# Lalwaniamisha789/Implementation-of-Neural-LDPC-Decoders-with-Degree-Specific-Weight-Sharing-and-RCQ-Quantization

Measured on AMD Instinct MI355X. Metric: decoded codewords/sec at fixed iters; achieved HBM GB/s vs peak, higher is better.
Workload: dtype f32

## Files before the change

### implementation-of-neural-ldpc-decoders-with-degree-specific-weight-sharing-and-rcq-quantization_amd/csrc/ldpc_resident.hip

```cpp
#pragma once

#include "ldpc_kernels.hip"
#include "ldpc_resident_geom.h"

namespace ldpc {

struct ResidentPlan {
    int n, m, S, max_dc, max_dv;
    int mstride;
    const uint8_t *dc_s;
    const uint8_t *gsz;
    int any_split;
    int par_words;
    int par_shift;
    const uint16_t *cvar;
    const uint16_t *bslot;
    const uint16_t *bslot_c;
    const uint16_t *oaslot;
    const uint32_t *vmeta;
    const uint2 *vslot_lo;
    const uint2 *vslot_hi;
    int n_hi;
    const uint16_t *inv_perm_v;
    int n_pos;
// ... 722 lines not shown
        }
    }
}

__device__ __forceinline__ uint4 plan_unpack(const uint2 &p)
{
    return make_uint4(p.x & 0xffffu, p.x >> 16, p.y & 0xffffu, p.y >> 16);
}

template <int G, int MODE, typename T, int DMAX = 8>
__device__ __forceinline__ void res_var_dispatch(unsigned char *smem, T *__restrict__ llr_s,
                                                 uint8_t *__restrict__ bits_s, int q, int dv, const uint4 &slo,
                                                 const uint4 &shi, T a, unsigned emask, const ParScatter &ps,
                                                 Pack<T, G> *lreg = nullptr)
{
#define LDPC_RV(D) \
    case D: if constexpr (D <= DMAX) res_var_body<G, D, MODE, T>(smem, llr_s, bits_s, q, slo, shi, a, emask, ps, lreg); break;
    switch (dv) {
        LDPC_RV(0) LDPC_RV(1) LDPC_RV(2) LDPC_RV(3) LDPC_RV(4) LDPC_RV(5) LDPC_RV(6) LDPC_RV(7) LDPC_RV(8)
    default: break;
    }
#undef LDPC_RV
}

template <typename T, int G>
struct ResVarState {
    unsigned meta[kResRegVars];
    uint2 plo[kResRegVars];
    uint2 phi0;
    Pack<T, G> l[kResRegVars];
    unsigned cells;
};

template <int G, int MODE, typename T, int R>
__device__ __forceinline__ void res_var_round_cpt(const ResidentPlan &pl, unsigned char *smem, const T *__restrict__ alpha_glb,
                                                  unsigned emask, int tid, int nt, ResVarState<T, G> &st)
{
    constexpr int DMAX = R == 0 ? 8 : 4;
    const unsigned cd = (st.cells >> (8 * R)) & 0xffu;
    if (cd == kCellEmpty) return;
    const int q = tid + R * nt;
    const uint4 slo = plan_unpack(st.plo[R]), shi = R == 0 ? plan_unpack(st.phi0) : make_uint4(0, 0, 0, 0);
    T a = (T)0;
    if (MODE == 0) a = alpha_glb[pl.vmeta[q] >> 8];
    const ParScatter ps{};
    if (cd == kCellMixed) {
        res_var_dispatch<G, MODE, T, DMAX>(smem, nullptr, nullptr, q, (int)(pl.vmeta[q] & 0xffu), slo, shi, a, emask, ps,
                                           &st.l[R]);
        return;
    }
    if ((cd & kCellHoles) && st.plo[R].y == kResHole) return;
#define LDPC_RVU(D) \
    case D: if constexpr (D <= DMAX) res_var_body<G, D, MODE, T>(smem, nullptr, nullptr, q, slo, shi, a, emask, ps, &st.l[R]); break;
    switch (cd & 0xfu) {
        LDPC_RVU(1) LDPC_RVU(2) LDPC_RVU(3) LDPC_RVU(4) LDPC_RVU(5) LDPC_RVU(6) LDPC_RVU(7) LDPC_RVU(8)
    default: break;
    }
#undef LDPC_RVU
}

template <int G, int MODE, typename T>
__device__ __forceinline__ void res_var_phase_cpt(const ResidentPlan &pl, unsigned char *smem, const T *__restrict__ alpha_glb,
                                                  unsigned emask, int tid, int nt, ResVarState<T, G> &st)
{
#pragma unroll
    for (int r = 0; r < kResRegVars; ++r) asm volatile("" : "+v"(st.plo[r].x), "+v"(st.plo[r].y));
    asm volatile("" : "+v"(st.phi0.x), "+v"(st.phi0.y));
    static_assert(kResRegVars == 4, "four rounds");
    res_var_round_cpt<G, MODE, T, 0>(pl, smem, alpha_glb, emask, tid, nt, st);
    res_var_round_cpt<G, MODE, T, 1>(pl, smem, alpha_glb, emask, tid, nt, st);
    res_var_round_cpt<G, MODE, T, 2>(pl, smem, alpha_glb, emask, tid, nt, st);
    res_var_round_cpt<G, MODE, T, 3>(pl, smem, alpha_glb, emask, tid, nt, st);
}

template <int G, int MODE, typename T>
__device__ __forceinline__ void res_var_phase_reg(const ResidentPlan &pl, unsigned char *smem,
                                                  T *__restrict__ llr_s, uint8_t *__restrict__ bits_s,
                                                  const T *__restrict__ alpha_lds,
                                                  const T *__restrict__ alpha_glb, unsigned emask,
                                                  int tid, int nt, ResVarState<T, G> &st, const ParScatter &ps)
{
#pragma unroll
    for (int r = 0; r < kResRegVars; ++r) asm volatile("" : "+v"(st.meta[r]), "+v"(st.plo[r].x), "+v"(st.plo[r].y));
    asm volatile("" : "+v"(st.phi0.x), "+v"(st.phi0.y));
#pragma unroll
    for (int r = 0; r < kResRegVars; ++r) {
        const int q = tid + r * nt;
        if (__builtin_amdgcn_readfirstlane(q - (tid & 63)) >= pl.n) break;
        if (q < pl.n) {
            const unsigned meta = st.meta[r];
            const uint4 slo = plan_unpack(st.plo[r]), shi = r == 0 ? plan_unpack(st.phi0) : make_uint4(0, 0, 0, 0);
            T a = (T)0;
            if (MODE == 0 || MODE == 4) a = alpha_lds ? alpha_lds[meta >> 8] : alpha_glb[meta >> 8];
            res_var_dispatch<G, MODE, T>(smem, llr_s, bits_s, q, (int)(meta & 0xffu), slo, shi, a, emask, ps, &st.l[r]);
        }
    }
}

template <int G, int MODE, typename T, bool REG, bool CPT = false>
__device__ __forceinline__ void res_var_phase(const ResidentPlan &pl, unsigned char *smem,
                                              T *__restrict__ llr_s, uint8_t *__restrict__ bits_s,
                                              const T *__restrict__ alpha_lds,
                                              const T *__restrict__ alpha_glb, unsigned emask,
                                              int tid, int nt, ResVarState<T, G> &st,
                                              const ParScatter ps = ParScatter{})
{
    if constexpr (CPT) {
        static_assert(REG && (MODE == 0 || MODE == 2 || MODE == 9), "compact: fixed-T register-state modes");
        res_var_phase_cpt<G, MODE, T>(pl, smem, alpha_glb, emask, tid, nt, st);
        return;
    } else if constexpr (REG) {
        res_var_phase_reg<G, MODE, T>(pl, smem, llr_s, bits_s, alpha_lds, alpha_glb, emask, tid, nt, st, ps);
        return;
    }
    const int n = pl.n, n_hi = pl.n_hi;
    const int hi_last = (n_hi > 0 ? n_hi : 1) - 1;
    int q = tid;
    unsigned meta = 0;
    uint2 plo = make_uint2(0, 0), phi = make_uint2(0, 0);
    if (q < n) {
        meta = pl.vmeta[q];
        plo = pl.vslot_lo[q];
        phi = pl.vslot_hi[min(q, hi_last)];
    }
    while (q < n) {
        const int qn = q + nt;
        unsigned metan;
        uint2 plon, phin;
        {
            const unsigned qc = (unsigned)min(qn, n - 1), qh = min(qc, (unsigned)hi_last);
            metan = *reinterpret_cast<const uint32_t *>(reinterpret_cast<const char *>(pl.vmeta) + (size_t)(qc << 2));
            plon = *reinterpret_cast<const uint2 *>(reinterpret_cast<const char *>(pl.vslot_lo) + (size_t)(qc << 3));
            phin = *reinterpret_cast<const uint2 *>(reinterpret_cast<const char *>(pl.vslot_hi) + (size_t)(qh << 3));
        }
        const int dv = (int)(meta & 0xffu);
        const uint4 slo = plan_unpack(plo), shi = plan_unpack(phi);
        T a = (T)0;
        if (MODE == 0 || MODE == 4) a = alpha_lds ? alpha_lds[meta >> 8] : alpha_glb[meta >> 8];
        res_var_dispatch<G, MODE, T>(smem, llr_s, bits_s, q, dv, slo, shi, a, emask, ps);
        q = qn; meta = metan; plo = plon; phi = phin;
    }
}

template <int G, bool SPLIT>
__device__ __forceinline__ void res_syndrome_phase(const ResidentPlan &pl, const uint8_t *__restrict__ bits_s,
                                                   unsigned *sh_unsat, int tid, int nt)
{
    unsigned acc = 0;
    for (int p = tid; p < pl.m; p += nt) {
        const int dc = pl.dc_s[p];
        int dcw;
        unsigned x = 0;
        if (wave_uniform(dc, dcw)) {
#pragma unroll 8
            for (int t = 0; t < dcw; ++t) x ^= bits_s[pl.cvar[t * pl.mstride + p]];
        } else {
            for (int t = 0; t < dc; ++t) x ^= bits_s[pl.cvar[t * pl.mstride + p]];
        }
        if constexpr (SPLIT) x = group_xor(pl.gsz[p], x);
        acc |= x;
    }
    if (acc) atomicOr(sh_unsat, acc);
}

template <int G, bool SPLIT>
__device__ __forceinline__ void res_parity_reduce(const ResidentPlan &pl, unsigned par_off, unsigned *sh_unsat, int tid, int nt)
{
    unsigned acc = 0;
    for (int p = tid; p < pl.m; p += nt) {
        unsigned x = lds_load<unsigned>(par_off + 4u * (unsigned)p);
        lds_store<unsigned>(par_off + 4u * (unsigned)p, 0u);
        if constexpr (SPLIT) x = group_xor(pl.gsz[p], x);
        acc |= x;
    }
    if (acc) atomicOr(sh_unsat, acc);
}

template <int G, typename T, bool SPLIT>
__device__ __forceinline__ void res_syndrome_slots(const ResidentPlan &pl, unsigned *sh_unsat, int tid, int nt)
{
    constexpr unsigned kSlot = sizeof(Pack<T, G>);
    unsigned acc = 0;
    for (int p = tid; p < pl.m; p += nt) {
        const int dc = pl.dc_s[p];
        int dcw;
        unsigned x = 0;
        if (wave_uniform(dc, dcw)) {
            int t = 0;
#pragma unroll 4
            for (; t + 1 < dcw; t += 2)
                x = __builtin_amdgcn_bitop3_b32(x, lds_load<unsigned>((unsigned)(t * pl.mstride + p) * kSlot),
                                                lds_load<unsigned>((unsigned)((t + 1) * pl.mstride + p) * kSlot), 0x96);
            if (t < dcw) x ^= lds_load<unsigned>((unsigned)(t * pl.mstride + p) * kSlot);
        } else {
            for (int t = 0; t < dc; ++t) x ^= lds_load<unsigned>((unsigned)(t * pl.mstride + p) * kSlot);
        }
        if constexpr (SPLIT) x = group_xor(pl.gsz[p], x);
        acc |= x;
    }
    if (acc) atomicOr(sh_unsat, acc);
}

constexpr int kEmit = 4;

template <int G>
__device__ __forceinline__ void res_store_packed(const ResidentArgs &a, long long b, int j, int n, bool neg)
{
    const unsigned long long m = __ballot(neg);
    const int lane = threadIdx.x & 63;
    const int base = j - lane;
    if (lane < 8 && base + 8 * lane < n) a.packed[(size_t)b * ((n + 7) / 8) + (base >> 3) + lane] = (uint8_t)(m >> (8 * lane));
}

template <int G, typename T>
__device__ __forceinline__ void res_emit(const ResidentPlan &pl, const ResidentArgs &a, const T *__restrict__ llr_s,
                                         long long b0, unsigned mask, int iters, unsigned unsat, int tid, int nt)
{
    using P = Pack<T, G>;
    T *posterior = reinterpret_cast<T *>(a.posterior);
    const int n = pl.n;
    if (a.posterior || a.bits || a.packed) {
        for (int j0 = tid; j0 < n; j0 += kEmit * nt) {
            unsigned ip[kEmit];
#pragma unroll
            for (int k = 0; k < kEmit; ++k) ip[k] = (j0 + k * nt < n) ? pl.inv_perm_v[j0 + k * nt] : 0u;
#pragma unroll
            for (int k = 0; k < kEmit; ++k) {
                const int j = j0 + k * nt;
                if (j - (tid & 63) >= n) break;
                const bool in = j < n;
                const P p = reinterpret_cast<const P *>(llr_s)[ip[k]];
#pragma unroll
                for (int g = 0; g < G; ++g) {
                    if (!((mask >> g) & 1u)) continue;
                    if (in && a.posterior) res_stream_store(&posterior[(size_t)(b0 + g) * n + j], p.x[g]);
                    if (in && a.bits) res_stream_store(&a.bits[(size_t)(b0 + g) * n + j], p.x[g] < (T)0 ? 1 : 0);
                    if (a.packed) res_store_packed<G>(a, b0 + g, j, n, in && p.x[g] < (T)0);
                }
            }
        }
    }
    if (tid == 0) {
#pragma unroll
        for (int g = 0; g < G; ++g) {
            if (!((mask >> g) & 1u)) continue;
            if (a.iterations) a.iterations[b0 + g] = iters;
            if (a.success) a.success[b0 + g] = (uint8_t)(((unsat >> g) & 1u) ? 0 : 1);
        }
    }
}

template <int G>
__device__ __forceinline__ void res_emit_bits(const ResidentPlan &pl, const ResidentArgs &a, const uint8_t *__restrict__ bits_s,
                                              long long b0, unsigned mask, int iters, unsigned unsat, int tid, int nt)
{
    const int n = pl.n;
    if (a.bits || a.packed) {
        for (int j0 = tid; j0 < n; j0 += kEmit * nt) {
            unsigned ip[kEmit];
#pragma unroll
            for (int k = 0; k < kEmit; ++k) ip[k] = (j0 + k * nt < n) ? pl.inv_perm_v[j0 + k * nt] : 0u;
#pragma unroll
            for (int k = 0; k < kEmit; ++k) {
                const int j = j0 + k * nt;
                if (j - (tid & 63) >= n) break;
                const bool in = j < n;
                const unsigned bb = bits_s[ip[k]];
#pragma unroll
                for (int g = 0; g < G; ++g) {
                    if (!((mask >> g) & 1u)) continue;
                    const unsigned bit = (bb >> g) & 1u;
                    if (in && a.bits) res_stream_store(&a.bits[(size_t)(b0 + g) * n + j], (int)bit);
                    if (a.packed) res_store_packed<G>(a, b0 + g, j, n, in && bit != 0);
                }
            }
        }
    }
    if (tid == 0) {
#pragma unroll
        for (int g = 0; g < G; ++g) {
            if (!((mask >> g) & 1u)) continue;
            if (a.iterations) a.iterations[b0 + g] = iters;
            if (a.success) a.success[b0 + g] = (uint8_t)(((unsat >> g) & 1u) ? 0 : 1);
        }
    }
}

template <int G, typename T>
__device__ __forceinline__ void res_dump_c2v(const ResidentPlan &pl, const ResidentArgs &a, long long b0, unsigned mask,
                                             int tid, int nt)
{
    using P = Pack<T, G>;
    T *out = reinterpret_cast<T *>(a.dbg_c2v);
    for (int s = tid; s < pl.S; s += nt) {
        const unsigned e = pl.edge_of_slot[s];
        if (e == 0xffffffffu) continue;
        const P v = lds_load<P>((unsigned)s * (unsigned)sizeof(P));
#pragma unroll
        for (int g = 0; g < G; ++g)
            if ((mask >> g) & 1u) out[(size_t)(b0 + g) * pl.E + e] = v.x[g];
    }
}

constexpr int kResMaxThreads = 1024;
constexpr int kResMinWaves = 4;
template <int G, int FORM, bool BPC, int NL, int MS, int ES, typename T = float, bool SPLIT = false, bool REG = false,
          bool CPT = false>
__global__ __launch_bounds__(CPT ? kResCptThreads : kResMaxThreads, CPT ? kResCptWaves : kResMinWaves)
void resident_decode(ResidentPlan pl, ResidentArgs a)
{
    static_assert(!CPT || (REG && !ES && !SPLIT && std::is_same<T, float>::value), "compact: fixed-T fp32 REG kernels only");
    extern __shared__ __align__(16) unsigned char res_smem[];
    if (__builtin_amdgcn_groupstaticsize() != 0) __builtin_trap();
    constexpr int GE = G * (int)(sizeof(T) / 4);
    const int n_alpha_lds = a.alpha_in_lds ? a.T * a.n_alpha * (int)(sizeof(T) / 4) : 0;
    T *llr_s = reinterpret_cast<T *>(res_smem + (CPT ? 0 : res_off_llr(pl.S, GE)));
    T *alpha_s = reinterpret_cast<T *>(res_smem + res_off_alpha(pl.S, pl.n, GE));
    uint8_t *bits_s = res_smem + res_off_bits(pl.S, pl.n, GE, n_alpha_lds);
    unsigned *sh_unsat = reinterpret_cast<unsigned *>(res_smem + (CPT ? res_cpt_off_flag(pl.S, GE)
                                                                        : res_off_flag(pl.S, pl.n, GE, n_alpha_lds)));
    ParScatter ps, psf;
    if (pl.par_words) {
        psf.par_off = (unsigned)res_off_par(pl.S, pl.n, GE, n_alpha_lds);
        psf.shift = (unsigned)pl.par_shift;
        psf.mask = (unsigned)pl.mstride - 1u;
        if (ES) ps = psf;
    }
    const T *g_llr = reinterpret_cast<const T *>(a.llr);
    const T *g_beta = reinterpret_cast<const T *>(a.beta);
    const T *g_alpha = reinterpret_cast<const T *>(a.alpha);
    const T *g_oms_alpha = reinterpret_cast<const T *>(a.oms_alpha);
    using P = Pack<T, G>;
    const int tid = threadIdx.x, nt = blockDim.x, n = pl.n;
    const long long b0 = (long long)blockIdx.x * G;
    constexpr unsigned kAll = (1u << G) - 1u;

    constexpr int kPro = 4;
    for (int j0 = tid; j0 < n; j0 += kPro * nt) {
        unsigned ip[kPro];
        P v[kPro];
#pragma unroll
        for (int k = 0; k < kPro; ++k) {
            const int j = j0 + k * nt;
            ip[k] = 0;
            if (j < n) {
                ip[k] = pl.inv_perm_v[j];
#pragma unroll
                for (int g = 0; g < G; ++g)
                    v[k].x[g] = (b0 + g < a.batch) ? res_stream_load(&g_llr[(size_t)(b0 + g) * n + j]) : (T)1;
            }
        }
#pragma unroll
        for (int k = 0; k < kPro; ++k)
            if (j0 + k * nt < n) reinterpret_cast<P *>(llr_s)[ip[k]] = v[k];
    }
    for (int k = tid; k < (a.alpha_in_lds ? a.T * a.n_alpha : 0); k += nt) alpha_s[k] = g_alpha[k];
    if (tid == 0) { sh_unsat[0] = 0; sh_unsat[1] = 0; }
    for (int k = tid; k < pl.par_words; k += nt) lds_store<unsigned>(psf.par_off + 4u * (unsigned)k, 0u);
    __syncthreads();
    ResVarState<T, G> st{};
    if constexpr (CPT) {
        st.cells = pl.vcell[__builtin_amdgcn_readfirstlane(tid) >> 6];
        const P *L = reinterpret_cast<const P *>(llr_s);
#pragma unroll
        for (int r = 0; r < kResRegVars; ++r) {
            const int q = tid + r * nt;
            if (q < pl.n_pos) st.l[r] = L[q];
            if ((st.cells >> (8 * r)) & 0xffu) {
                st.plo[r] = pl.vslot_lo[q];
                if (r == 0 && q < pl.n_hi) st.phi0 = pl.vslot_hi[q];
            }
        }
        __syncthreads();
#pragma unroll
        for (int r = 0; r < kResRegVars; ++r) {
            const unsigned cd = (st.cells >> (8 * r)) & 0xffu;
            if (cd == kCellEmpty) continue;
            const int q = tid + r * nt;
            int dv = (int)(cd & 0xfu);
            if (cd == kCellMixed) dv = (int)(pl.vmeta[q] & 0xffu);
            else if ((cd & kCellHoles) && st.plo[r].y == kResHole) dv = 0;
            const uint4 slo = plan_unpack(st.plo[r]), shi = r == 0 ? plan_unpack(st.phi0) : make_uint4(0, 0, 0, 0);
            const unsigned off[8] = {slo.x, slo.y, slo.z, slo.w, shi.x, shi.y, shi.z, shi.w};
            P l = st.l[r];
            if (a.T == 0) {
#pragma unroll
                for (int g = 0; g < G; ++g) l.x[g] = (T)0;
            }
#pragma unroll
            for (int e = 0; e < (r == 0 ? 8 : 4); ++e)
                if (e < dv) lds_store<P>(off[e], l);
        }
    } else if constexpr (REG) {
        const P *L = reinterpret_cast<const P *>(llr_s);
#pragma unroll
        for (int r = 0; r < kResRegVars; ++r) {
            const int q = tid + r * nt;
            if (q < n) {
                st.meta[r] = pl.vmeta[q];
                st.plo[r] = pl.vslot_lo[q];
                if (r == 0 && q < pl.n_hi) st.phi0 = pl.vslot_hi[q];
                st.l[r] = L[q];
            }
        }
#pragma unroll
        for (int r = 0; r < kResRegVars; ++r) {
            if (tid + r * nt < n) {
                const uint4 slo = plan_unpack(st.plo[r]), shi = r == 0 ? plan_unpack(st.phi0) : make_uint4(0, 0, 0, 0);
                const unsigned off[8] = {slo.x, slo.y, slo.z, slo.w, shi.x, shi.y, shi.z, shi.w};
                const int dv = (int)(st.meta[r] & 0xffu);
                P l = st.l[r];
                if constexpr (!std::is_same<T, float>::value) {
#pragma unroll
                    for (int g = 0; g < G; ++g) l.x[g] = __builtin_canonicalize(l.x[g]);
                }
                if (a.T == 0) {
#pragma unroll
                    for (int g = 0; g < G; ++g) l.x[g] = (T)0;
                }
#pragma unroll
                for (int e = 0; e < 8; ++e)
                    if (e < dv) lds_store<P>(off[e], l);
            }
        }
    } else {
        const P *L = reinterpret_cast<const P *>(llr_s);
        for (int q0 = tid; q0 < n; q0 += kPro * nt) {
            int dvk[kPro];
            uint2 plo[kPro], phi[kPro];
#pragma unroll
            for (int k = 0; k < kPro; ++k) {
                const int q = q0 + k * nt;
                dvk[k] = 0;
                plo[k] = make_uint2(0, 0);
                phi[k] = make_uint2(0, 0);
                if (q < n) {
                    dvk[k] = (int)(pl.vmeta[q] & 0xffu);
                    plo[k] = pl.vslot_lo[q];
                    if (q < pl.n_hi) phi[k] = pl.vslot_hi[q];
                }
            }
#pragma unroll
            for (int k = 0; k < kPro; ++k) {
                const int q = q0 + k * nt;
                if (q < n) {
                    const uint4 slo = plan_unpack(plo[k]), shi = plan_unpack(phi[k]);
                    const unsigned off[8] = {slo.x, slo.y, slo.z, slo.w, shi.x, shi.y, shi.z, shi.w};
                    P l = L[q];
                    if constexpr (!std::is_same<T, float>::value) {
#pragma unroll
                        for (int g = 0; g < G; ++g) l.x[g] = __builtin_canonicalize(l.x[g]);
                    }
                    if (a.T == 0) {
#pragma unroll
                        for (int g = 0; g < G; ++g) l.x[g] = (T)0;
                    }
#pragma unroll
                    for (int e = 0; e < 8; ++e)
                        if (e < dvk[k]) lds_store<P>(off[e], l);
                }
            }
        }
    }
    unsigned chk_cells = 0;
    if constexpr (CPT) chk_cells = pl.ccell[__builtin_amdgcn_readfirstlane(tid) >> 6];
    const int dc_pre = tid < pl.m ? pl.dc_s[tid] : 0;
    T b_pre = (BPC && tid < pl.m && a.T > 0) ? g_beta[pl.bslot_c[tid]] : (T)0;
    __syncthreads();

    unsigned done = 0;
#pragma unroll
    for (int g = 0; g < G; ++g)
        if (b0 + g >= a.batch) done |= 1u << g;

    for (int it = 0; it < a.T; ++it) {
        const T *beta_row = g_beta + (size_t)it * a.n_beta;
        const T *oa_row = a.oms_alpha ? g_oms_alpha + (size_t)it * a.n_oms_alpha : nullptr;
        const float *thr = FORM == FORM_RCQ ? a.thr + (size_t)a.q_of_iter[it] * a.n_levels : nullptr;
        const T *alpha_lds = a.alpha_in_lds ? alpha_s + it * a.n_alpha : nullptr;
        const T *alpha_glb = g_alpha + (size_t)it * a.n_alpha;
        res_check_phase<G, FORM, BPC, NL, MS, T, SPLIT, CPT>(pl, res_smem, beta_row, oa_row, thr, a.n_levels,
                                                             a.rcq_zero0 != 0, dc_pre, b_pre, tid, nt, chk_cells);
        if (BPC && tid < pl.m && it + 1 < a.T)
            b_pre = g_beta[(size_t)(it + 1) * a.n_beta + pl.bslot_c[tid]];
        __syncthreads();
        if (ES && !a.posterior) {
            const bool last = it == a.T - 1;
            if (last) res_var_phase<G, 1, T, REG>(pl, res_smem, llr_s, bits_s, (const T *)nullptr, (const T *)nullptr, 0u, tid, nt, st, ps);
            else if (a.unit_alpha) res_var_phase<G, 6, T, REG>(pl, res_smem, llr_s, bits_s, (const T *)nullptr, (const T *)nullptr, 0u, tid, nt, st, ps);
            else res_var_phase<G, 4, T, REG>(pl, res_smem, llr_s, bits_s, alpha_lds, alpha_glb, 0u, tid, nt, st, ps);
            __syncthreads();
            unsigned *su = sh_unsat + (it & 1);
            if (ps.par_off) res_parity_reduce<G, SPLIT>(pl, ps.par_off, su, tid, nt);
            else res_syndrome_phase<G, SPLIT>(pl, bits_s, su, tid, nt);
            __syncthreads();
            const unsigned unsat = *su;
            if (tid == 0) sh_unsat[(it + 1) & 1] = 0;
            const unsigned newly = ~unsat & ~done & kAll;
            if (newly) {
                res_emit_bits<G>(pl, a, bits_s, b0, newly, it + 1, 0u, tid, nt);
                done |= newly;
                if (done == kAll) return;
                __syncthreads();
            }
            continue;
        }
        if (ES) {
            res_var_phase<G, 1, T, REG>(pl, res_smem, llr_s, bits_s, (const T *)nullptr, (const T *)nullptr, 0u, tid, nt, st, ps);
            __syncthreads();
            unsigned *su = sh_unsat + (it & 1);
            if (ps.par_off) res_parity_reduce<G, SPLIT>(pl, ps.par_off, su, tid, nt);
            else res_syndrome_phase<G, SPLIT>(pl, bits_s, su, tid, nt);
            __syncthreads();
            const unsigned unsat = *su;
            if (tid == 0) sh_unsat[(it + 1) & 1] = 0;
            const unsigned newly = ~unsat & ~done & kAll;
            if (newly) {
                if (a.dbg_c2v) res_dump_c2v<G, T>(pl, a, b0, newly, tid, nt);
                res_var_phase<G, 1, T, REG>(pl, res_smem, llr_s, bits_s, (const T *)nullptr, (const T *)nullptr, newly, tid, nt, st);
                __syncthreads();
                res_emit<G, T>(pl, a, llr_s, b0, newly, it + 1, 0u, tid, nt);
                done |= newly;
                if (done == kAll) return;
                __syncthreads();
            }
        }
        if (it != a.T - 1) {
            if (a.unit_alpha) res_var_phase<G, 2, T, REG, CPT>(pl, res_smem, llr_s, bits_s, (const T *)nullptr, (const T *)nullptr, 0u, tid, nt, st);
            else res_var_phase<G, 0, T, REG, CPT>(pl, res_smem, llr_s, bits_s, alpha_lds, alpha_glb, 0u, tid, nt, st);
            __syncthreads();
        }
    }

    const unsigned open = ~done & kAll;
    if (!open) return;
    if (a.dbg_c2v) {
        unsigned real = 0;
#pragma unroll
        for (int g = 0; g < G; ++g)
            if (b0 + g < a.batch) real |= 1u << g;
        res_dump_c2v<G, T>(pl, a, b0, open & real, tid, nt);
        __syncthreads();
    }
    if (ES && !a.posterior && a.T > 0) {
        res_emit_bits<G>(pl, a, bits_s, b0, open, a.T, kAll, tid, nt);
        return;
    }
    const bool scatter = !ES && !CPT && psf.par_off != 0;
    if (ES) res_var_phase<G, 1, T, REG>(pl, res_smem, llr_s, bits_s, (const T *)nullptr, (const T *)nullptr, open, tid, nt, st);
    else if (scatter) res_var_phase<G, 1, T, REG>(pl, res_smem, llr_s, bits_s, (const T *)nullptr, (const T *)nullptr, open, tid, nt, st, psf);
    else res_var_phase<G, CPT ? 9 : 8, T, REG, CPT>(pl, res_smem, llr_s, bits_s, (const T *)nullptr, (const T *)nullptr, open, tid, nt, st);
    __syncthreads();
    unsigned unsat = kAll;
    if (!ES) {
        if (scatter) res_parity_reduce<G, SPLIT>(pl, psf.par_off, sh_unsat, tid, nt);
        else res_syndrome_slots<G, T, SPLIT>(pl, sh_unsat, tid, nt);
        __syncthreads();
        unsat = *sh_unsat;
    }
    if constexpr (CPT) {
#pragma unroll
        for (int r = 0; r < kResRegVars; ++r)
            if (tid + r * nt < pl.n_pos) reinterpret_cast<P *>(llr_s)[tid + r * nt] = st.l[r];
        __syncthreads();
    }
    res_emit<G, T>(pl, a, llr_s, b0, open, a.T, unsat, tid, nt);
}

}
```

Baseline: 36.53 million.

## Specialize compact kernel prologue/epilogue with hoisted plan loads and full-block fast paths

For compact (CPT) kernels, plan metadata loads (vslot, cells, dc, beta column) are hoisted before the first barrier and issued alongside the LLR staging. Full blocks use an unguarded, fixed-row staging and emit path with scalar row pointers and clamped indices. The exit path also gets a dedicated syndrome check and a register-to-LDS writeback, selected per form. The aim is to cut prologue and epilogue latency and branch overhead, at the cost of more code specialization and careful bounds clamping.

After: 37.20 million (median of 6 runs). 1.9% higher.

```diff
diff --git a/implementation-of-neural-ldpc-decoders-with-degree-specific-weight-sharing-and-rcq-quantization_amd/csrc/ldpc_resident.hip b/implementation-of-neural-ldpc-decoders-with-degree-specific-weight-sharing-and-rcq-quantization_amd/csrc/ldpc_resident.hip
--- a/implementation-of-neural-ldpc-decoders-with-degree-specific-weight-sharing-and-rcq-quantization_amd/csrc/ldpc_resident.hip
+++ b/implementation-of-neural-ldpc-decoders-with-degree-specific-weight-sharing-and-rcq-quantization_amd/csrc/ldpc_resident.hip
@@ -1048,6 +1048,213 @@
     }
 }
 
+constexpr int kCptRows = 4;
+constexpr unsigned kCptEntry = 1u;
+constexpr unsigned kCptInit = 2u;
+constexpr unsigned kCptExit = 4u;
+constexpr unsigned res_cpt_forms(int form, bool bpc, int nl)
+{
+    if (form == FORM_OMS) return bpc ? kCptEntry | kCptInit : kCptInit;
+    if (form == FORM_RCQ && nl == 4 && !bpc) return kCptEntry | kCptInit;
+    return kCptEntry | kCptInit | kCptExit;
+}
+static_assert(kCptRows == kResRegVars, "the staging rows are the register rounds");
+
+template <typename X>
+__device__ __forceinline__ const X *res_at(const X *base, unsigned i)
+{
+    return reinterpret_cast<const X *>(reinterpret_cast<const char *>(base) + (size_t)(i * (unsigned)sizeof(X)));
+}
+template <typename X>
+__device__ __forceinline__ X *res_at(X *base, unsigned i)
+{
+    return reinterpret_cast<X *>(reinterpret_cast<char *>(base) + (size_t)(i * (unsigned)sizeof(X)));
+}
+
+template <typename X>
+__device__ __forceinline__ X *res_row(X *base, size_t elems)
+{
+    unsigned long long row = (unsigned long long)(base + elems);
+    asm volatile("" : "+s"(row));
+    return (X *)(__attribute__((address_space(1))) X *)row;
+}
+
+template <int G>
+__device__ __forceinline__ bool res_cpt_full_block(const ResidentPlan &pl, const ResidentArgs &a, long long b0)
+{
+    int rows = kCptRows - 1;
+    asm volatile("" : "+s"(rows));
+    return b0 + G <= a.batch && pl.n > rows * kResCptThreads;
+}
+
+template <int G, bool BPC>
+__device__ __forceinline__ void res_cpt_plan_loads(const ResidentPlan &pl, int tid, unsigned wbase, ResVarState<float, G> &st,
+                                                   unsigned &chk_cells, int &dc_pre, unsigned &bcol)
+{
+    const unsigned lane = (unsigned)tid - wbase;
+    st.cells = pl.vcell[wbase >> 6];
+    chk_cells = pl.ccell[wbase >> 6];
+#pragma unroll
+    for (int r = 0; r < kResRegVars; ++r) {
+        const unsigned qb = ((st.cells >> (8 * r)) & 0xffu) ? wbase + (unsigned)(r * kResCptThreads) : 0u;
+        st.plo[r] = *res_at(pl.vslot_lo, qb + lane);
+    }
+    st.phi0 = *res_at(pl.vslot_hi, min((unsigned)tid, (unsigned)max(pl.n_hi, 1) - 1u));
+    const unsigned pc = min((unsigned)tid, (unsigned)pl.m - 1u);
+    dc_pre = *res_at(pl.dc_s, pc);
+    bcol = BPC ? *res_at(pl.bslot_c, pc) : 0u;
+}
+
+template <int G>
+__device__ __forceinline__ void res_cpt_stage_llrs(const ResidentPlan &pl, const float *__restrict__ g_llr, long long b0, int tid,
+                                                   unsigned wbase)
+{
+    using P = Pack<float, G>;
+    constexpr int K = kCptRows, NT = kResCptThreads;
+    const unsigned n = (unsigned)pl.n;
+    const float *row[G];
+#pragma unroll
+    for (int g = 0; g < G; ++g) row[g] = res_row(g_llr, (size_t)(b0 + g) * n);
+    unsigned ip[K];
+    P v[K];
+#pragma unroll
+    for (int k = 0; k < K - 1; ++k) {
+        const unsigned j = (unsigned)tid + (unsigned)(k * NT);
+        ip[k] = *res_at(pl.inv_perm_v, j);
+#pragma unroll
+        for (int g = 0; g < G; ++g) v[k].x[g] = res_stream_load(res_at(row[g], j));
+    }
+    const bool last = wbase + (unsigned)((K - 1) * NT) < n;
+    if (last) {
+        const unsigned j = min((unsigned)tid + (unsigned)((K - 1) * NT), n - 1u);
+        ip[K - 1] = *res_at(pl.inv_perm_v, j);
+#pragma unroll
+        for (int g = 0; g < G; ++g) v[K - 1].x[g] = res_stream_load(res_at(row[g], j));
+    }
+#pragma unroll
+    for (int k = 0; k < K - 1; ++k) lds_store<P>(ip[k] * (unsigned)sizeof(P), v[k]);
+    if (last) lds_store<P>(ip[K - 1] * (unsigned)sizeof(P), v[K - 1]);
+}
+
+template <int G, int R>
+__device__ __forceinline__ void res_cpt_init_round(const ResidentPlan &pl, const ResVarState<float, G> &st, int tid, bool zero)
+{
+    using P = Pack<float, G>;
+    const unsigned cd = (st.cells >> (8 * R)) & 0xffu;
+    if (cd == kCellEmpty) return;
+    const uint4 slo = plan_unpack(st.plo[R]), shi = R == 0 ? plan_unpack(st.phi0) : make_uint4(0, 0, 0, 0);
+    const unsigned off[8] = {slo.x, slo.y, slo.z, slo.w, shi.x, shi.y, shi.z, shi.w};
+    P l = st.l[R];
+    if (zero) {
+#pragma unroll
+        for (int g = 0; g < G; ++g) l.x[g] = 0.0f;
+    }
+    if (cd == kCellMixed) {
+        const int dv = (int)(pl.vmeta[tid + R * kResCptThreads] & 0xffu);
+#pragma unroll
+        for (int e = 0; e < (R == 0 ? 8 : 4); ++e)
+            if (e < dv) lds_store<P>(off[e], l);
+        return;
+    }
+    if ((cd & kCellHoles) && st.plo[R].y == kResHole) return;
+    const int dv = (int)(cd & 0xfu);
+#pragma unroll
+    for (int e = 0; e < (R == 0 ? 8 : 4); ++e)
+        if (e < dv) lds_store<P>(off[e], l);
+}
+
+template <int G, int MS>
+__device__ __forceinline__ void res_cpt_syndrome_slots(unsigned cw, int dc, unsigned *sh_unsat, int tid)
+{
+    constexpr unsigned kSlot = sizeof(Pack<float, G>), stride = (unsigned)MS * kSlot;
+    auto body = [&]() {
+        unsigned x = 0;
+        res_walk_edges((unsigned)tid * kSlot, stride, chk_lo(cw), chk_spread(cw), dc, [&](unsigned addr, auto kc) {
+            constexpr int K = decltype(kc)::value;
+            unsigned v[K];
+#pragma unroll
+            for (int k = 0; k < K; ++k) v[k] = lds_load<unsigned>(addr + k * stride);
+            if constexpr (K == 1) {
+                x ^= v[0];
+            } else {
+#pragma unroll
+                for (int k = 0; k < K; k += 2) x = __builtin_amdgcn_bitop3_b32(x, v[k], v[k + 1], 0x96);
+            }
+        });
+        if (x) atomicOr(sh_unsat, x);
+    };
+    const int lanes = chk_lanes(cw);
+    if (lanes == 64) body();
+    else if ((tid & 63) < lanes) body();
+}
+
+template <int G>
+__device__ __forceinline__ void res_cpt_emit(const ResidentPlan &pl, const ResidentArgs &a, long long b0, const unsigned (&ip)[kCptRows],
+                                             int iters, unsigned unsat, int tid, unsigned wbase)
+{
+    using P = Pack<float, G>;
+    constexpr int K = kCptRows, NT = kResCptThreads;
+    const unsigned n = (unsigned)pl.n, jl = (unsigned)tid + (unsigned)((K - 1) * NT), jwl = wbase + (unsigned)((K - 1) * NT);
+    const bool last = jwl < n;
+    const bool part = jwl + 64u > n;
+    if (a.posterior || a.bits || a.packed) {
+        P p[K];
+#pragma unroll
+        for (int k = 0; k < K - 1; ++k) p[k] = lds_load<P>(ip[k] * (unsigned)sizeof(P));
+        if (last) p[K - 1] = lds_load<P>(ip[K - 1] * (unsigned)sizeof(P));
+        if (a.posterior) {
+            float *row[G];
+#pragma unroll
+            for (int g = 0; g < G; ++g) {
+                row[g] = res_row(a.posterior, (size_t)(b0 + g) * n);
+#pragma unroll
+                for (int k = 0; k < K - 1; ++k) res_stream_store(res_at(row[g], (unsigned)tid + (unsigned)(k * NT)), p[k].x[g]);
+            }
+            if (last && (!part || jl < n)) {
+#pragma unroll
+                for (int g = 0; g < G; ++g) res_stream_store(res_at(row[g], jl), p[K - 1].x[g]);
+            }
+        }
+        if (a.bits) {
+            int *row[G];
+#pragma unroll
+            for (int g = 0; g < G; ++g) {
+                row[g] = res_row(a.bits, (size_t)(b0 + g) * n);
+#pragma unroll
+                for (int k = 0; k < K - 1; ++k)
+                    res_stream_store(res_at(row[g], (unsigned)tid + (unsigned)(k * NT)), p[k].x[g] < 0.0f ? 1 : 0);
+            }
+            if (last && (!part || jl < n)) {
+#pragma unroll
+                for (int g = 0; g < G; ++g) res_stream_store(res_at(row[g], jl), p[K - 1].x[g] < 0.0f ? 1 : 0);
+            }
+        }
+        if (a.packed) {
+            const unsigned lane = (unsigned)tid - wbase, nb = (n + 7u) >> 3;
+#pragma unroll
+            for (int g = 0; g < G; ++g) {
+                uint8_t *row = res_row(a.packed, (size_t)(b0 + g) * nb);
+#pragma unroll
+                for (int k = 0; k < K - 1; ++k) {
+                    const unsigned long long m = __ballot(p[k].x[g] < 0.0f);
+                    if (lane < 8) *res_at(row, ((wbase + (unsigned)(k * NT)) >> 3) + lane) = (uint8_t)(m >> (8 * lane));
+                }
+                if (last) {
+                    const unsigned long long m = __ballot(jl < n && p[K - 1].x[g] < 0.0f);
+                    if (lane < 8 && jwl + 8 * lane < n) *res_at(row, (jwl >> 3) + lane) = (uint8_t)(m >> (8 * lane));
+                }
+            }
+        }
+    }
+    if (tid == 0) {
+#pragma unroll
+        for (int g = 0; g < G; ++g) {
+            if (a.iterations) a.iterations[b0 + g] = iters;
+            if (a.success) a.success[b0 + g] = (uint8_t)(((unsat >> g) & 1u) ? 0 : 1);
+        }
+    }
+}
+
 constexpr int kResMaxThreads = 1024;
 constexpr int kResMinWaves = 4;
 template <int G, int FORM, bool BPC, int NL, int MS, int ES, typename T = float, bool SPLIT = false, bool REG = false,
@@ -1061,12 +1268,12 @@
     constexpr int GE = G * (int)(sizeof(T) / 4);
     const int n_alpha_lds = a.alpha_in_lds ? a.T * a.n_alpha * (int)(sizeof(T) / 4) : 0;
     T *llr_s = reinterpret_cast<T *>(res_smem + (CPT ? 0 : res_off_llr(pl.S, GE)));
-    T *alpha_s = reinterpret_cast<T *>(res_smem + res_off_alpha(pl.S, pl.n, GE));
-    uint8_t *bits_s = res_smem + res_off_bits(pl.S, pl.n, GE, n_alpha_lds);
+    T *alpha_s = CPT ? nullptr : reinterpret_cast<T *>(res_smem + res_off_alpha(pl.S, pl.n, GE));
+    uint8_t *bits_s = CPT ? nullptr : res_smem + res_off_bits(pl.S, pl.n, GE, n_alpha_lds);
     unsigned *sh_unsat = reinterpret_cast<unsigned *>(res_smem + (CPT ? res_cpt_off_flag(pl.S, GE)
                                                                         : res_off_flag(pl.S, pl.n, GE, n_alpha_lds)));
     ParScatter ps, psf;
-    if (pl.par_words) {
+    if (!CPT && pl.par_words) {
         psf.par_off = (unsigned)res_off_par(pl.S, pl.n, GE, n_alpha_lds);
         psf.shift = (unsigned)pl.par_shift;
         psf.mask = (unsigned)pl.mstride - 1u;
@@ -1082,7 +1289,19 @@
     constexpr unsigned kAll = (1u << G) - 1u;
 
     constexpr int kPro = 4;
-    for (int j0 = tid; j0 < n; j0 += kPro * nt) {
+    ResVarState<T, G> st{};
+    unsigned chk_cells = 0;
+    int dc_cpt = 0;
+    unsigned bcol_cpt = 0;
+    bool cpt_fast = false;
+    constexpr unsigned EE = CPT ? res_cpt_forms(FORM, BPC, NL) : 0u;
+    if constexpr ((EE & kCptEntry) != 0) {
+        const unsigned wbase = (unsigned)__builtin_amdgcn_readfirstlane(tid) & ~63u;
+        res_cpt_plan_loads<G, BPC>(pl, tid, wbase, st, chk_cells, dc_cpt, bcol_cpt);
+        cpt_fast = res_cpt_full_block<G>(pl, a, b0);
+        if (cpt_fast) res_cpt_stage_llrs<G>(pl, g_llr, b0, tid, wbase);
+    }
+    for (int j0 = tid; j0 < (cpt_fast ? 0 : n); j0 += kPro * nt) {
         unsigned ip[kPro];
         P v[kPro];
 #pragma unroll
@@ -1100,42 +1319,65 @@
         for (int k = 0; k < kPro; ++k)
             if (j0 + k * nt < n) reinterpret_cast<P *>(llr_s)[ip[k]] = v[k];
     }
-    for (int k = tid; k < (a.alpha_in_lds ? a.T * a.n_alpha : 0); k += nt) alpha_s[k] = g_alpha[k];
+    if constexpr (!CPT) {
+        for (int k = tid; k < (a.alpha_in_lds ? a.T * a.n_alpha : 0); k += nt) alpha_s[k] = g_alpha[k];
+    }
     if (tid == 0) { sh_unsat[0] = 0; sh_unsat[1] = 0; }
-    for (int k = tid; k < pl.par_words; k += nt) lds_store<unsigned>(psf.par_off + 4u * (unsigned)k, 0u);
+    if constexpr (!CPT) {
+        for (int k = tid; k < pl.par_words; k += nt) lds_store<unsigned>(psf.par_off + 4u * (unsigned)k, 0u);
+    }
+    int dc_pre = 0;
+    T b_pre = (T)0;
+    if constexpr ((EE & kCptEntry) != 0) {
+        dc_pre = dc_cpt;
+        if (BPC && a.T > 0) b_pre = *res_at(g_beta, bcol_cpt);
+    }
     __syncthreads();
-    ResVarState<T, G> st{};
     if constexpr (CPT) {
-        st.cells = pl.vcell[__builtin_amdgcn_readfirstlane(tid) >> 6];
-        const P *L = reinterpret_cast<const P *>(llr_s);
-#pragma unroll
-        for (int r = 0; r < kResRegVars; ++r) {
-            const int q = tid + r * nt;
-            if (q < pl.n_pos) st.l[r] = L[q];
-            if ((st.cells >> (8 * r)) & 0xffu) {
-                st.plo[r] = pl.vslot_lo[q];
-                if (r == 0 && q < pl.n_hi) st.phi0 = pl.vslot_hi[q];
+        if constexpr ((EE & kCptEntry) != 0) {
+#pragma unroll
+            for (int r = 0; r < kResRegVars; ++r)
+                st.l[r] = lds_load<P>(min((unsigned)tid + (unsigned)(r * kResCptThreads), (unsigned)pl.n_pos - 1u) * (unsigned)sizeof(P));
+        } else {
+            st.cells = pl.vcell[__builtin_amdgcn_readfirstlane(tid) >> 6];
+            const P *L = reinterpret_cast<const P *>(llr_s);
+#pragma unroll
+            for (int r = 0; r < kResRegVars; ++r) {
+                const int q = tid + r * nt;
+                if (q < pl.n_pos) st.l[r] = L[q];
+                if ((st.cells >> (8 * r)) & 0xffu) {
+                    st.plo[r] = pl.vslot_lo[q];
+                    if (r == 0 && q < pl.n_hi) st.phi0 = pl.vslot_hi[q];
+                }
             }
         }
         __syncthreads();
-#pragma unroll
-        for (int r = 0; r < kResRegVars; ++r) {
-            const unsigned cd = (st.cells >> (8 * r)) & 0xffu;
-            if (cd == kCellEmpty) continue;
-            const int q = tid + r * nt;
-            int dv = (int)(cd & 0xfu);
-            if (cd == kCellMixed) dv = (int)(pl.vmeta[q] & 0xffu);
-            else if ((cd & kCellHoles) && st.plo[r].y == kResHole) dv = 0;
-            const uint4 slo = plan_unpack(st.plo[r]), shi = r == 0 ? plan_unpack(st.phi0) : make_uint4(0, 0, 0, 0);
-            const unsigned off[8] = {slo.x, slo.y, slo.z, slo.w, shi.x, shi.y, shi.z, shi.w};
-            P l = st.l[r];
-            if (a.T == 0) {
-#pragma unroll
-                for (int g = 0; g < G; ++g) l.x[g] = (T)0;
-            }
-#pragma unroll
-            for (int e = 0; e < (r == 0 ? 8 : 4); ++e)
-                if (e < dv) lds_store<P>(off[e], l);
+        if constexpr ((EE & kCptInit) != 0) {
+            static_assert(kResRegVars == 4, "four rounds");
+            res_cpt_init_round<G, 0>(pl, st, tid, a.T == 0);
+            res_cpt_init_round<G, 1>(pl, st, tid, a.T == 0);
+            res_cpt_init_round<G, 2>(pl, st, tid, a.T == 0);
+            res_cpt_init_round<G, 3>(pl, st, tid, a.T == 0);
+        } else {
+#pragma unroll
+            for (int r = 0; r < kResRegVars; ++r) {
+                const unsigned cd = (st.cells >> (8 * r)) & 0xffu;
+                if (cd == kCellEmpty) continue;
+                const int q = tid + r * nt;
+                int dv = (int)(cd & 0xfu);
+                if (cd == kCellMixed) dv = (int)(pl.vmeta[q] & 0xffu);
+                else if ((cd & kCellHoles) && st.plo[r].y == kResHole) dv = 0;
+                const uint4 slo = plan_unpack(st.plo[r]), shi = r == 0 ? plan_unpack(st.phi0) : make_uint4(0, 0, 0, 0);
+                const unsigned off[8] = {slo.x, slo.y, slo.z, slo.w, shi.x, shi.y, shi.z, shi.w};
+                P l = st.l[r];
+                if (a.T == 0) {
+#pragma unroll
+                    for (int g = 0; g < G; ++g) l.x[g] = (T)0;
+                }
+#pragma unroll
+                for (int e = 0; e < (r == 0 ? 8 : 4); ++e)
+                    if (e < dv) lds_store<P>(off[e], l);
+            }
         }
     } else if constexpr (REG) {
         const P *L = reinterpret_cast<const P *>(llr_s);
@@ -1208,10 +1450,11 @@
             }
         }
     }
-    unsigned chk_cells = 0;
-    if constexpr (CPT) chk_cells = pl.ccell[__builtin_amdgcn_readfirstlane(tid) >> 6];
-    const int dc_pre = tid < pl.m ? pl.dc_s[tid] : 0;
-    T b_pre = (BPC && tid < pl.m && a.T > 0) ? g_beta[pl.bslot_c[tid]] : (T)0;
+    if constexpr ((EE & kCptEntry) == 0) {
+        if constexpr (CPT) chk_cells = pl.ccell[__builtin_amdgcn_readfirstlane(tid) >> 6];
+        dc_pre = tid < pl.m ? pl.dc_s[tid] : 0;
+        b_pre = (BPC && tid < pl.m && a.T > 0) ? g_beta[pl.bslot_c[tid]] : (T)0;
+    }
     __syncthreads();
 
     unsigned done = 0;
@@ -1296,6 +1539,34 @@
     if (ES) res_var_phase<G, 1, T, REG>(pl, res_smem, llr_s, bits_s, (const T *)nullptr, (const T *)nullptr, open, tid, nt, st);
     else if (scatter) res_var_phase<G, 1, T, REG>(pl, res_smem, llr_s, bits_s, (const T *)nullptr, (const T *)nullptr, open, tid, nt, st, psf);
     else res_var_phase<G, CPT ? 9 : 8, T, REG, CPT>(pl, res_smem, llr_s, bits_s, (const T *)nullptr, (const T *)nullptr, open, tid, nt, st);
+    if constexpr ((EE & kCptExit) != 0) {
+        unsigned ip[kCptRows] = {};
+        cpt_fast = res_cpt_full_block<G>(pl, a, b0);
+        const unsigned wbase = (unsigned)__builtin_amdgcn_readfirstlane(tid) & ~63u;
+        if (cpt_fast) {
+#pragma unroll
+            for (int k = 0; k < kCptRows; ++k)
+                ip[k] = *res_at(pl.inv_perm_v, min((unsigned)tid + (unsigned)(k * kResCptThreads), (unsigned)n - 1u));
+        }
+        __syncthreads();
+        res_cpt_syndrome_slots<G, MS>(chk_cells, dc_pre, sh_unsat, tid);
+        __syncthreads();
+        const unsigned unsat = *sh_unsat;
+#pragma unroll
+        for (int r = 0; r < kResRegVars; ++r) {
+            const unsigned cd = (st.cells >> (8 * r)) & 0xffu;
+            const unsigned q = (unsigned)tid + (unsigned)(r * kResCptThreads);
+            if (cd == kCellEmpty) continue;
+            if (cd != kCellMixed && !(cd & kCellHoles)) lds_store<P>(q * (unsigned)sizeof(P), st.l[r]);
+            else if (q < (unsigned)pl.n_pos) lds_store<P>(q * (unsigned)sizeof(P), st.l[r]);
+        }
+        __syncthreads();
+#pragma unroll
+        for (int k = 0; k < kCptRows; ++k) asm volatile("" : "+v"(ip[k]));
+        if (cpt_fast) res_cpt_emit<G>(pl, a, b0, ip, a.T, unsat, tid, wbase);
+        else res_emit<G, T>(pl, a, llr_s, b0, open, a.T, unsat, tid, nt);
+        return;
+    }
     __syncthreads();
     unsigned unsat = kAll;
     if (!ES) {
```
